# damemi/odigos

Measured on AMD Instinct MI355X. Metric: spans/sec processed (whole node) at 1/2/4/8 MI355X; % of HBM roofline, higher is better.
Workload: dtype u8; 1 GPU; C4: fused odigossampling -> odigosurltemplate -> odigostrafficmetrics, 100M spans in total (all on one GPU at N=1; ~100M/N per GPU, trace-id all-to-all over RCCL at N>1); spans_per_gpu=100000000, spans_total=100000000, template_form=refs, seed=219545604, parallelism=dp1: independent span shards, no data-path collective

## Files before the change

### odigos_amd/csrc/engine.cpp

```cpp
#include <hip/hip_runtime.h>

#include <algorithm>
#include <map>
#include <cstdio>
#include <cstdlib>
#include <cstring>
#include <mutex>
#include <string>
#include <unordered_map>
#include <vector>

#include "../../include/odigos_amd.h"
#include "config.hpp"
#include "devcfg.hpp"
#include "engine_internal.hpp"
#include "kernels.hpp"
#include "blob.hpp"
#include "regex_dfa.hpp"

namespace ose {

thread_local std::string g_last_error;

int fail(int code, const std::string& msg) {
// ... 134 lines not shown
    if (w->table) (void)hipFree(w->table);
    if (w->dup_bkt) (void)hipFree(w->dup_bkt);
    if (w->dup_bkt_count) (void)hipFree(w->dup_bkt_count);
    if (w->runs) (void)hipFree(w->runs);
    if (w->run_count) (void)hipFree(w->run_count);
    if (w->attr_bits) (void)hipFree(w->attr_bits);
    if (w->ep_planes) (void)hipFree(w->ep_planes);
    if (w->svc_local) (void)hipFree(w->svc_local);
    for (void* f : w->fold)
      if (f) (void)hipFree(f);
    if (w->pending) (void)hipEventDestroy(w->pending);
    if (w->dup_host) (void)hipHostFree(w->dup_host);
    if (w->dup_ready) (void)hipEventDestroy(w->dup_ready);
    if (w->fork) (void)hipEventDestroy(w->fork);
    if (w->join) (void)hipEventDestroy(w->join);
    delete w;
  }
}

hipEvent_t Engine::take_event() {
  if (!event_pool.empty()) {
    hipEvent_t ev = event_pool.back();
    event_pool.pop_back();
    return ev;
  }
  hipEvent_t ev = nullptr;
  (void)hipEventCreate(&ev);
  return ev;
}
void Engine::prof_begin(const char* name, hipStream_t st, Timed& t) {
// ... 46 lines not shown
  if (w->pending_set) (void)hipStreamWaitEvent(st, w->pending, 0);
  return w;
}
void Engine::return_unused_ws(Workspace* w) {
  std::lock_guard<std::mutex> g(mu);
  w->captured = false;
  free_ws.push_back(w);
}
void Engine::release_ws(Workspace* w, hipStream_t st) {
  if (w->captured) return;
  if (!w->pending) (void)hipEventCreateWithFlags(&w->pending, hipEventDisableTiming);
  w->pending_set = w->pending && hipEventRecord(w->pending, st) == hipSuccess;
  std::lock_guard<std::mutex> g(mu);
  free_ws.push_back(w);
}
hipStream_t Engine::take_stream() {
  std::lock_guard<std::mutex> g(mu);
  if (!free_streams.empty()) {
    hipStream_t s = free_streams.back();
    free_streams.pop_back();
    return s;
  }
  hipStream_t s = nullptr;
  if (hipStreamCreateWithFlags(&s, hipStreamNonBlocking) != hipSuccess) return nullptr;
  streams.push_back(s);
  return s;
}
void Engine::give_stream(hipStream_t s) {
  std::lock_guard<std::mutex> g(mu);
  free_streams.push_back(s);
}

int Workspace::reserve(size_t bytes) {
  if (bytes <= cap) return 0;
  if (captured) return fail(OSE_ENOMEM, "workspace too small inside a hipGraph capture: call ose_reserve first");
  if (dev) HIP_TRY(hipFree(dev));
  dev = nullptr;
  cap = 0;
  size_t want = std::max<size_t>(bytes, 1 << 20);
// ... 39 lines not shown
  (void)hipDeviceSynchronize();
  delete e;
}

int upload(const std::vector<uint8_t>& host, uint8_t** dev) {
  HIP_TRY(hipMalloc(dev, host.size()));
  HIP_TRY(hipMemcpy(*dev, host.data(), host.size(), hipMemcpyHostToDevice));
  return 0;
}

static size_t align_up(size_t x, size_t a) { return (x + a - 1) / a * a; }

int run_url_back(Engine* e, const UrlKernelArgs& a, hipStream_t st);

int run_url(Engine* e, const ose_columns* c, const ose_outputs* o, hipStream_t st, Workspace* ws, size_t ws_off = 0,
            UrlKernelArgs* front = nullptr, bool refs = false, uint32_t grid_mult = 1) {
  if (!e->has_url) return fail(OSE_EINVAL, "odigosurltemplate is not configured on this engine");
  if (!c->url_flags || !c->kind || !c->path || !c->arena || !o->url_out || !o->tmpl || !o->tmpl_arena)
    return fail(OSE_EINVAL, "TEMPLATE stage needs url_flags, kind, path, arena, url_out, tmpl, tmpl_arena");
  if (e->url_needs_resource && (!c->resource || !c->res_url_ok))
    return fail(OSE_EINVAL, "include/exclude configured: resource and res_url_ok columns are required");
  if (c->res_url_ok && !c->resource) return fail(OSE_EINVAL, "res_url_ok needs the resource column");
  if (o->tmpl_arena_cap > 0xFFFFFFFFull) return fail(OSE_ERANGE, "tmpl_arena_cap exceeds the 32-bit offset range");
  uint64_t n = c->n_spans;
  const uint32_t groups = (uint32_t)((n + kUrlGroup - 1) / kUrlGroup);
  const uint32_t scan_tiles = (groups + kUrlScanTile - 1) / kUrlScanTile;
  const size_t off_bump = 16, off_asum = 24, off_sst = 32, zero_bytes = off_sst + 8 * (size_t)scan_tiles;
  const size_t off_len = align_up(zero_bytes, 256), off_meta = off_len + 4 * n;
  const size_t off_code = align_up(off_meta + 4 * n, 8);
  const size_t off_gsum = off_code + 8 * n, off_gbase = off_gsum + 8 * (size_t)groups;
  const size_t off_gscr = off_gbase + 8 * (size_t)groups;
// ... 44 lines not shown
  a.slow_groups = reinterpret_cast<uint32_t*>(base + off_slow);
  a.unplanned_count = reinterpret_cast<uint32_t*>(base + 12);
  a.unplanned = reinterpret_cast<uint32_t*>(base + off_unpl);
  HIP_TRY(hipMemsetAsync(base, 0, zero_bytes, st));
  a.used = o->tmpl_arena_used;
#if OSE_DIAG
  if (const char* ab = getenv("OSE_URL_ABLATE")) a.ablate = (uint32_t)strtoul(ab, nullptr, 0);
#endif
  a.plan_grid_mult = refs ? grid_mult : 1u;
  a.scr_region = (scr_bytes / std::max<uint32_t>(1, url_plan_waves(a))) & ~15ull;
  a.plan_waves = url_plan_waves(a);
  a.refs_chunk = url_refs_chunk(o->tmpl_arena_cap, a.plan_waves);
  if (front) *front = a;
  if (n == 0) {
    if (o->tmpl_arena_used) HIP_TRY(hipMemsetAsync(o->tmpl_arena_used, 0, 8, st));
    return 0;
  }
  if (a.ablate & 512) {
    a.dbg = reinterpret_cast<uint64_t*>(base + off_dbg);
    HIP_TRY(hipMemsetAsync(a.dbg, 0, 256, st));
  }
  Engine::Timed tm{};
  e->prof_begin("url_plan_kernel", st, tm);
  launch_url_plan(a, st);
  HIP_TRY(hipGetLastError());
  e->prof_end(tm, st);
  e->prof_begin("url_plan_slow_kernel", st, tm);
  launch_url_plan_slow(a, st);
  HIP_TRY(hipGetLastError());
  e->prof_end(tm, st);
  e->prof_begin("url_scan_kernel", st, tm);
  launch_url_scan(a, st);
  HIP_TRY(hipGetLastError());
  e->prof_end(tm, st);
  e->prof_begin("url_emit_slow_kernel", st, tm);
  launch_url_emit_slow(a, st);
  HIP_TRY(hipGetLastError());
  e->prof_end(tm, st);
  if (front) {
    *front = a;
    return 0;
  }
  return run_url_back(e, a, st);
}

int run_url_back(Engine* e, const UrlKernelArgs& a, hipStream_t st) {
  if (a.n_spans == 0) return 0;
  Engine::Timed tm{};
  e->prof_begin("url_copy_kernel", st, tm);
  launch_url_copy(a, st);
  HIP_TRY(hipGetLastError());
  e->prof_end(tm, st);
  if (a.ablate & 512) {
    uint64_t h[16];
    uint32_t cnt[4];
    HIP_TRY(hipMemcpyAsync(h, a.dbg, sizeof h, hipMemcpyDeviceToHost, st));
    HIP_TRY(hipMemcpyAsync(cnt, a.scan_counter, sizeof cnt, hipMemcpyDeviceToHost, st));
    HIP_TRY(hipStreamSynchronize(st));
    const double wp = h[3] ? (double)h[3] : 1.0, we = h[6] ? (double)h[6] : 1.0;
    (void)we;
    fprintf(stderr, "url clocks/wave: plan[stage %.0f bitmaps %.0f plan %.0f assemble+store %.0f]\n", h[0] / wp,
            h[1] / wp, h[2] / wp, h[5] / wp);
    fprintf(stderr, "url plan list clocks/wave: enumerate %.0f classify %.0f fold %.0f\n", h[13] / wp, h[14] / wp,
            h[15] / wp);
    fprintf(stderr, "url groups: %llu, slow (K3s) %u, unplanned (K1b) %u\n", (unsigned long long)((a.n_spans + 63) / 64),
            cnt[1], cnt[3]);
    fprintf(stderr, "url_plan_slow_kernel slowest block clocks: config %llu whole %llu plan_path %llu\n",
// ... 30 lines not shown
  if (mask & OSE_STAGE_TEMPLATE) {
    need = std::max(need, url_off + url_workspace_bytes(n, c->arena_bytes));
    size_off = align_up(url_off + url_workspace_bytes(n, c->arena_bytes), 256);
  }
  if (mask & OSE_STAGE_SIZE) need = std::max(need, size_off + size_scratch_bytes(c->n_scopes, c->n_resources));
  int rc = ws->reserve(need);
  std::function<int()> sample_tail;
  UrlKernelArgs ua{};
  hipStream_t ust = nullptr;
  static const bool one_stream = getenv("OSE_ONE_STREAM") != nullptr;
  constexpr uint64_t kForkSpans = 1u << 20;
  const uint32_t plan_groups = (uint32_t)((n + kUrlGroup - 1) / kUrlGroup);
  if (!one_stream && !rc && defer && n >= kForkSpans) {
    if (!ws->fork) (void)hipEventCreateWithFlags(&ws->fork, hipEventDisableTiming);
    if (!ws->join) (void)hipEventCreateWithFlags(&ws->join, hipEventDisableTiming);
    if (ws->fork && ws->join) ust = e->take_stream();
    if (ust && (hipEventRecord(ws->fork, st) != hipSuccess || hipStreamWaitEvent(ust, ws->fork, 0) != hipSuccess)) {
      e->give_stream(ust);
      ust = nullptr;
    }
  }
  const bool tmpl = !rc && (mask & OSE_STAGE_TEMPLATE);
  ws->beside_url = ust && tmpl;
  if (ust && tmpl)
    rc = run_url(e, c, o, ust, ws, url_off, &ua, (mask & OSE_STAGE_TEMPLATE_REFS) != 0, url_plan_grid_mult(plan_groups, true));
  if (!rc && (mask & OSE_STAGE_SAMPLE)) rc = run_sampling(e, c, o, group_mode, rnd, st, ws, gate_on_host ? &sample_tail : nullptr);
  if (sample_tail && !defer) {
    rc = sample_tail();
    sample_tail = nullptr;
  }
  if (!ust && tmpl && !rc)
    rc = run_url(e, c, o, st, ws, url_off, &ua, (mask & OSE_STAGE_TEMPLATE_REFS) != 0, url_plan_grid_mult(plan_groups));
  if (sample_tail) {
    const int trc = sample_tail();
    if (!rc) rc = trc;
  }
  if (ust) {
    const hipError_t je = hipEventRecord(ws->join, ust);
    const hipError_t jw = je == hipSuccess ? hipStreamWaitEvent(st, ws->join, 0) : je;
    if (jw != hipSuccess) {
      (void)hipStreamSynchronize(ust);
      if (!rc) rc = fail(OSE_EDEVICE, std::string("URL stream join: ") + hipGetErrorString(jw));
    }
    e->give_stream(ust);
  }
  SizeKernelArgs sa{};
  bool size_on = false;
  if (!rc && (mask & OSE_STAGE_SIZE)) rc = prepare_size(e, c, o, mask, group_mode, rnd, st, ws, size_off, sa, size_on);
  if (!rc && tmpl) {
    if (size_on && n > 0 && !(OSE_DIAG && getenv("OSE_NO_FUSED_SIZE"))) {
      sa.kept_partials = size_partials_of(ws, size_off, c->n_scopes, c->n_resources);
      sa.n_kept_partials = url_copy_blocks(ua.n_groups);
      ua.fuse_size = 1;
      ua.size_partials = const_cast<uint32_t*>(sa.kept_partials);
      ua.sz = sa;
    }
    rc = run_url_back(e, ua, st);
  }
  if (!rc && size_on) rc = run_size_tail(e, sa, st);
  ws->beside_url = false;
  e->release_ws(ws, st);
  return rc;
}

}

using namespace ose;

extern "C" {

const char* ose_last_error(void) { return g_last_error.c_str(); }

uint64_t ose_dropped_errors(char* last, size_t cap) {
  std::lock_guard<std::mutex> g(g_dropped_mu);
// ... 312 lines not shown
```

### odigos_amd/csrc/engine_internal.hpp

```cpp
#pragma once
#include <hip/hip_runtime.h>

#include <atomic>
#include <cstdint>
#include <functional>
#include <mutex>
#include <string>
#include <unordered_map>
#include <vector>

#include "../../include/odigos_amd.h"
#include "config.hpp"

namespace ose {

int fail(int code, const std::string& msg);
struct Engine;
int bind_device(const Engine* e);
int ensure_device();
void engine_retain(Engine* e);
void engine_unref(Engine* e);
void note_dropped_error(const char* where, hipError_t err);
struct LastErrorScope {
  const char* where;
// ... 35 lines not shown
  uint64_t fold_cap = 0;
  int reserve_fold(uint64_t n_spans);
  uint64_t* attr_bits = nullptr;
  uint64_t attr_bits_cap = 0;
  int reserve_attr(uint64_t n_spans);
  uint64_t* ep_planes = nullptr;
  uint64_t ep_planes_cap = 0;
  ose_columns spill_cols{};
  uint32_t* svc_local = nullptr;
  uint64_t svc_local_cap = 0;
  ose_columns local_cols{};
  int reserve_svc_local(uint64_t n_resources);
  int reserve_ep_planes(uint64_t words);
  uint32_t* dup_host = nullptr;
  hipEvent_t dup_ready = nullptr;
  hipEvent_t fork = nullptr, join = nullptr;
  bool beside_url = false;
};

struct Engine {
  std::atomic<int> refs{1};
  std::atomic<bool> closed{false};
  int device = 0;
  UrlTemplateConfig url;
  SamplingConfig sampling;
  TrafficMetricsConfig traffic;
  bool has_url = false, has_sampling = false, has_traffic = false;
  enum : uint32_t { kOptOtlpGpuChain = 1, kOptOtlpHostResources = 2, kOptOtlpHostScopes = 4, kOptEncodeHost = 8 };
  std::atomic<uint32_t> options{0};
  bool option(uint32_t o) const { return (options.load(std::memory_order_relaxed) & o) != 0; }
  bool url_needs_resource = false;
// ... 83 lines not shown
```

### odigos_amd/csrc/size_kernel.hip

```cpp
#include <hip/hip_runtime.h>

#include <algorithm>
#include <cstdint>
#include <cstdlib>

#include "device_common.hpp"
#include "kernels.hpp"
#include "size_device.hpp"

namespace ose {
namespace {

using namespace sizedev;
constexpr int kSThreads = 256;
constexpr uint32_t kLdsAttrsets = 2048;

__device__ __forceinline__ bool batch_dropped(const SizeKernelArgs& a) { return size_batch_dropped(a); }

__global__ __launch_bounds__(kSThreads) void size_span_kernel(SizeKernelArgs a) {
  if (batch_dropped(a)) return;
  __shared__ uint32_t wk[kSThreads / kWave];
  uint32_t kept_total = 0;
  const uint64_t stride = (uint64_t)gridDim.x * kSThreads;
  for (uint64_t base = (uint64_t)blockIdx.x * kSThreads; base < a.n_spans; base += 2 * stride) {
    const SpanCols x0 = size_span_load(a, base + threadIdx.x);
    const SpanCols x1 = size_span_load(a, base + stride + threadIdx.x);
    kept_total += size_span_finish(a, x0);
    if (base + stride < a.n_spans) kept_total += size_span_finish(a, x1);
  }
#pragma unroll
// ... 6 lines not shown
    if (k) atomicAdd((unsigned long long*)a.accepted, (unsigned long long)k);
  }
}

__device__ __forceinline__ void size_finish_res(const SizeKernelArgs& a, unsigned long long* hist, bool lds, uint32_t r,
                                                uint64_t body, uint32_t alive, bool had, uint32_t rsz, uint32_t set) {
  const bool removed = a.remove_empty && had && alive == 0;
  const uint64_t size = removed ? 0 : (uint64_t)rsz + body;
  if (a.res_bytes) a.res_bytes[r] = size;
  if (removed) return;
  const long long add = (long long)size * a.inverse;
  if (lds) atomicAdd(&hist[set], (unsigned long long)add);
  else atomicAdd((unsigned long long*)&a.attrset_bytes[set], (unsigned long long)add);
}

__global__ __launch_bounds__(kSThreads) void size_tail_kernel(SizeKernelArgs a) {
  __shared__ unsigned long long hist[kLdsAttrsets];
  __shared__ uint32_t wk[kSThreads / kWave];
  const bool lds = a.n_attrsets <= kLdsAttrsets;
  const int lane = threadIdx.x & 63;
  const uint64_t gstride = (uint64_t)gridDim.x * kSThreads;
  if (batch_dropped(a)) {
    if (a.res_bytes)
      for (uint64_t r = (uint64_t)blockIdx.x * kSThreads + threadIdx.x; r < a.n_resources; r += gstride) a.res_bytes[r] = 0;
    return;
  }
  if (lds)
    for (uint32_t k = threadIdx.x; k < a.n_attrsets; k += kSThreads) hist[k] = 0;
  __syncthreads();
  const uint32_t S = a.n_scopes, R = a.n_resources;
  if (S == 0) {
    for (uint64_t r = (uint64_t)blockIdx.x * kSThreads + threadIdx.x; r < R; r += gstride)
      size_finish_res(a, hist, lds, (uint32_t)r, 0, 0, false, a.res_size[r], a.res_attrset[r]);
  }
  for (uint64_t t0 = (uint64_t)blockIdx.x * kSThreads; t0 < S; t0 += gstride) {
    const uint64_t s = t0 + threadIdx.x;
    const uint64_t s0 = s - lane;
    const bool valid = s < S;
    uint32_t r = 0xFFFFFFFFu, alive = 0, had = 0;
    uint64_t contrib = 0;
    uint32_t nb = 0xFFFFFFFFu;
    if (valid) {
      r = a.scope_resource[s];
      const uint64_t sb = a.scope_body[s];
      const uint64_t body = sb & kSumMask;
      had = (sb >> kSumBits) != 0;
      alive = !a.remove_empty || !had || body != 0;
      if (alive) contrib = field_len((uint64_t)a.scope_size[s] + body);
      if (lane == 0 && s > 0) nb = a.scope_resource[s - 1];
    }
    uint32_t rsz = 0, rset = 0;
    if (valid) {
      rsz = a.res_size[r];
      rset = a.res_attrset[r];
    }
    const uint64_t vmask = __ballot(valid);
    if (!vmask) continue;
    const int lastv = 63 - __clzll((long long)vmask);
    uint32_t na = 0xFFFFFFFFu;
    if (lane == lastv && s + 1 < S) na = a.scope_resource[s + 1];
    uint64_t v = contrib;
    uint32_t c = alive;
    const bool tail = wave_seg_sum(r, valid, v, c);
    const uint32_t pr = dpp_mov<0x138>(r, r);
    const bool head = valid && (lane == 0 || pr != r);
    const uint64_t heads = __ballot(head);
    const uint64_t hadm = __ballot(had != 0);
    const uint64_t upto = ~0ull >> (63 - lane);
    const int start = 63 - __clzll((long long)(heads & upto));
    const uint32_t h = (hadm & upto & (~0ull << start)) ? 1u : 0u;
    const uint32_t r0 = __builtin_amdgcn_readfirstlane(r);
    const uint32_t rl = (uint32_t)__builtin_amdgcn_readlane((int)r, lastv);
    const uint32_t before = __builtin_amdgcn_readfirstlane(nb);
    const uint32_t after = (uint32_t)__builtin_amdgcn_readlane((int)na, lastv);
    const bool whole_head = s0 == 0 || before != r0;
    const bool whole_tail = s0 + lastv + 1 >= S || after != rl;
    const int end0 = __builtin_ctzll(__ballot(tail));
    const bool single = end0 == lastv;
    const bool cut = tail && ((start == 0 && !whole_head) || (lane == lastv && !whole_tail));
    if (tail && !cut) size_finish_res(a, hist, lds, r, v, c, h != 0, rsz, rset);
    if (valid && head) {
      const uint32_t prev = lane ? pr : (s0 == 0 ? 0xFFFFFFFFu : before);
      for (uint32_t g = prev + 1; g < r; g++) size_finish_res(a, hist, lds, g, 0, 0, false, a.res_size[g], a.res_attrset[g]);
    }
    if (valid && s + 1 == S)
      for (uint32_t g = r + 1; g < R; g++) size_finish_res(a, hist, lds, g, 0, 0, false, a.res_size[g], a.res_attrset[g]);
    const uint64_t w = s0 >> 6;
    const uint32_t ch0 = (uint32_t)__builtin_amdgcn_readlane((int)(c | (h << 30)), end0);
    const uint64_t v0 = ((uint64_t)(uint32_t)__builtin_amdgcn_readlane((int)(uint32_t)(v >> 32), end0) << 32) |
                        (uint32_t)__builtin_amdgcn_readlane((int)(uint32_t)v, end0);
    const uint32_t chl = (uint32_t)__builtin_amdgcn_readlane((int)(c | (h << 30)), lastv);
    const uint64_t vl = ((uint64_t)(uint32_t)__builtin_amdgcn_readlane((int)(uint32_t)(v >> 32), lastv) << 32) |
                        (uint32_t)__builtin_amdgcn_readlane((int)(uint32_t)v, lastv);
    if (lane == 0 && valid) {
      a.parts[2 * w] = SizePart{r0, ch0 | (whole_head ? 1u << 31 : 0u), v0};
      a.parts[2 * w + 1] = SizePart{rl, chl | (whole_tail ? 1u << 31 : 0u), vl};
      a.fix[w] = (!whole_head && (!single || whole_tail)) ? 1u : 0u;
    }
  }
  if (a.kept_partials) {
    uint32_t k = 0;
    for (uint32_t b = blockIdx.x * kSThreads + threadIdx.x; b < a.n_kept_partials; b += gridDim.x * kSThreads)
      k += a.kept_partials[b];
#pragma unroll
    for (int o = 32; o > 0; o >>= 1) k += __shfl_xor(k, o, kWave);
    if (lane == 0) wk[threadIdx.x >> 6] = k;
    __syncthreads();
    if (threadIdx.x == 0) {
      uint32_t t = 0;
      for (int q = 0; q < kSThreads / kWave; q++) t += wk[q];
      if (t) atomicAdd((unsigned long long*)a.accepted, (unsigned long long)t);
    }
  }
// ... 17 lines not shown
    alive += lp.ch & 0x3FFFFFFFu;
    had |= (lp.ch >> 30) & 1u;
    const SizePart fp = a.parts[2 * k];
    if (fp.r != r || (fp.ch >> 31)) break;
  }
  size_finish_res(a, nullptr, false, r, body, alive, had, a.res_size[r], a.res_attrset[r]);
}
}

void launch_size_spans(const SizeKernelArgs& a, hipStream_t st) {
  constexpr uint64_t cap = 1024;
  const uint64_t blocks = std::min<uint64_t>((a.n_spans + kSThreads - 1) / kSThreads, cap);
  if (blocks) hipLaunchKernelGGL(size_span_kernel, dim3((uint32_t)blocks), dim3(kSThreads), 0, st, a);
}
void launch_size_tail(const SizeKernelArgs& a, hipStream_t st) {
  uint64_t blocks = ((uint64_t)a.n_scopes + kSThreads - 1) / kSThreads;
#ifndef OSE_SIZE_TAIL_CAP
#define OSE_SIZE_TAIL_CAP 4096
#endif
  if (blocks > OSE_SIZE_TAIL_CAP) blocks = OSE_SIZE_TAIL_CAP;
  if (a.kept_partials) blocks = std::max<uint64_t>(blocks, std::min<uint32_t>(64, (a.n_kept_partials + 4095) / 4096));
  if (!blocks && a.n_resources) blocks = std::min<uint64_t>(((uint64_t)a.n_resources + kSThreads - 1) / kSThreads, 1024);
  if (blocks) hipLaunchKernelGGL(size_tail_kernel, dim3((uint32_t)blocks), dim3(kSThreads), 0, st, a);
}
void launch_size_fix(const SizeKernelArgs& a, hipStream_t st) {
  if (a.n_swin) hipLaunchKernelGGL(size_fix_kernel, dim3((a.n_swin + kSThreads - 1) / kSThreads), dim3(kSThreads), 0, st, a);
}

}
```

### odigos_amd/csrc/url_kernel.hip

```cpp
#include <hip/hip_runtime.h>

#include <algorithm>
#include <cstdlib>

#include "../../include/odigos_amd.h"
#include "device_common.hpp"
#include "kernels.hpp"
#include "size_device.hpp"
#include "url_classes.hpp"

#ifndef OSE_ASM_BATCH
#define OSE_ASM_BATCH 0
#endif

namespace ose {
namespace {

constexpr int kThreads = 256;
constexpr int kWaves = kThreads / kWave;
constexpr uint32_t kStage = 4 * 1024;

enum : uint32_t { M_NONE = 0, M_RENAME_SLASH, M_SLASH, M_RULE, M_DEFAULT, M_ORIG };

__device__ __forceinline__ bool is_digit(uint32_t c) { return c - '0' < 10u; }
// ... 1358 lines not shown
      if (!(a.ablate & 64))
        assemble_group((lds_out_u8*)sm.bm[wv], L, (uint32_t)(stage - (uint8_t*)&sm), sm.segs[wv], sm.cls[wv], sm.bn,
                       bn_src, p, seg_off, local, cfg.n_custom == 0);
      wave_lds_sync();
      uint4* dst = reinterpret_cast<uint4*>(a.scratch + region + scr_used);
      for (uint32_t k = lane; k < n16; k += kWave) {
        const u32x4 v = img4[k];
        dst[k] = make_uint4(v.x, v.y, v.z, v.w);
      }
      if (lane == 0) {
        a.group_sum[g] = sum;
        a.group_scr[g] = region + scr_used;
      }
      if (a.refs && i < a.n_spans) a.tmpl[i] = ose_strref{(uint32_t)(region + scr_used + local), p.len};
      scr_used += need;
    } else if (lane == 0) {
      a.group_sum[g] = sum;
      a.group_scr[g] = ~0ull;
      if (sum) a.slow_groups[atomicAdd(a.slow_count, 1u)] = g;
    }
    }
    if (tm) { const uint64_t t1 = clk(); t_emit += t1 - t0; t0 = t1; }
    if (!more) break;
    wave_lds_sync();
    pf = stage_dma(a.arena, np2 ? nxt.pr.off : ~0u, np2 ? nxt.pr.off + nxt.pr.len : 0u, sm.stage[wv]);
    g = g2;
  }
  if (tm && lane == 0) {
    atomicAdd((unsigned long long*)&a.dbg[0], (unsigned long long)t_stage);
    atomicAdd((unsigned long long*)&a.dbg[1], (unsigned long long)t_bm);
    atomicAdd((unsigned long long*)&a.dbg[2], (unsigned long long)t_plan);
    atomicAdd((unsigned long long*)&a.dbg[3], 1ull);
    atomicAdd((unsigned long long*)&a.dbg[5], (unsigned long long)t_emit);
    atomicAdd((unsigned long long*)&a.dbg[13], (unsigned long long)tt[0]);
// ... 55 lines not shown
  }
  __syncthreads();
  if (k < a.n_groups) a.group_base[k] = sb + prefix + wbase + incl - v;
}

struct CopyCols {
  uint32_t len;
  uint64_t base, gsum, so;
};
__device__ __forceinline__ CopyCols copy_cols(const UrlKernelArgs& a, uint32_t g, int lane) {
  CopyCols c{0, 0, 0, ~0ull};
  const uint64_t i = (uint64_t)g * kWave + lane;
  c.base = a.group_base[g];
  c.gsum = a.group_sum[g];
  c.so = a.group_scr[g];
  if (i < a.n_spans) c.len = a.plan_len[i];
  return c;
}
__device__ __forceinline__ void copy_round(uint8_t* gdst, uint32_t shift, uint64_t endb, uint32_t c0, uint32_t nchunk,
                                           const uint4& v, uint32_t& carry) {
  const int lane = threadIdx.x & 63;
  const uint32_t c = c0 + (uint32_t)lane;
  uint32_t pw = (uint32_t)__shfl_up((int)v.w, 1, kWave);
  if (lane == 0) pw = carry;
  carry = lane_value(v.w, kWave - 1);
  const uint32_t sh = 4 - shift;
  const uint32_t w0 = shift ? __builtin_amdgcn_alignbyte(v.x, pw, sh) : v.x;
  const uint32_t w1 = shift ? __builtin_amdgcn_alignbyte(v.y, v.x, sh) : v.y;
  const uint32_t w2 = shift ? __builtin_amdgcn_alignbyte(v.z, v.y, sh) : v.z;
  const uint32_t w3 = shift ? __builtin_amdgcn_alignbyte(v.w, v.z, sh) : v.w;
// ... 10 lines not shown
#pragma unroll
      for (uint32_t q = 0; q < 16; q++)
        if (b0 + q >= shift && b0 + q < endb) gdst[b0 + q] = (uint8_t)(ws[q >> 2] >> (8 * (q & 3)));
    }
  }
}
struct CopyJob {
  const uint4* src;
  uint8_t* gdst;
  uint32_t shift, n16, nchunk;
  uint64_t endb;
  bool on;
};
__device__ __forceinline__ CopyJob copy_job(const UrlKernelArgs& a, const CopyCols& c) {
  CopyJob j{};
  j.on = !a.refs && c.so != ~0ull && c.gsum != 0 && c.base + c.gsum <= a.out_cap;
  if (!j.on) return j;
  j.src = reinterpret_cast<const uint4*>(a.scratch + c.so);
  j.shift = (uint32_t)(c.base & 3);
  j.gdst = a.out_arena + (c.base - j.shift);
  j.endb = j.shift + c.gsum;
  j.n16 = (uint32_t)((c.gsum + 15) / 16);
  j.nchunk = (uint32_t)((j.endb + 15) / 16);
  return j;
}
__device__ __forceinline__ uint4 copy_load(const CopyJob& j, uint32_t c0) {
  const uint32_t c = c0 + (threadIdx.x & 63);
  return j.on && c < j.n16 ? j.src[c] : make_uint4(0, 0, 0, 0);
}
__device__ __forceinline__ void copy_rest(const CopyJob& j, uint4 v, uint32_t& carry) {
  copy_round(j.gdst, j.shift, j.endb, 0, j.nchunk, v, carry);
  for (uint32_t c0 = kWave; c0 < j.nchunk; c0 += kWave) {
    v = copy_load(j, c0);
    copy_round(j.gdst, j.shift, j.endb, c0, j.nchunk, v, carry);
  }
}
template <bool kSize>
__global__ __launch_bounds__(kThreads) __attribute__((amdgpu_waves_per_eu(kSize ? 5 : 6, 8))) void url_copy_kernel(UrlKernelArgs a) {
  const int lane = threadIdx.x & 63;
  const uint32_t stride = wave_stride();
  if (!kSize && a.refs) {
    for (uint64_t g0 = (uint64_t)wave_first_group() * kWave; g0 < a.n_groups; g0 += (uint64_t)stride * kWave) {
      const uint64_t gg = g0 + lane;
      const bool other = gg < a.n_groups && a.group_scr[gg] == ~0ull;
      for (uint64_t m = __ballot(other); m; m &= m - 1) {
        const uint32_t g = (uint32_t)(g0 + __builtin_ctzll(m));
        const CopyCols A = copy_cols(a, g, lane);
        uint32_t unused;
        const uint32_t la = wave_excl_scan(A.len, &unused);
        const uint64_t ia = (uint64_t)g * kWave + lane;
        if (ia < a.n_spans) a.tmpl[ia] = ose_strref{(uint32_t)(A.base + la), A.len};
      }
    }
    return;
  }
  uint32_t kept = 0;
  const bool sz_on = kSize && !sizedev::size_batch_dropped(a.sz);
  uint32_t g = wave_first_group();
  CopyCols An{0, 0, 0, ~0ull};
  sizedev::SpanCols xn{};
  if (g < a.n_groups) {
    An = copy_cols(a, g, lane);
    if (kSize && sz_on) xn = sizedev::size_span_load(a.sz, (uint64_t)g * kWave + lane, false);
  }
  for (; g < a.n_groups; g += stride) {
    const uint64_t ia = (uint64_t)g * kWave + lane;
    const CopyCols A = An;
    const sizedev::SpanCols x0 = xn;
    const bool more = g + stride < a.n_groups;
    if (more) {
      An = copy_cols(a, g + stride, lane);
      if (kSize && sz_on) xn = sizedev::size_span_load(a.sz, (uint64_t)(g + stride) * kWave + lane, false);
    }
    sizedev::SpanCols x = x0;
    uint32_t unused;
    const uint32_t la = wave_excl_scan(A.len, &unused);
    const CopyJob ja = copy_job(a, A);
    const uint4 va = copy_load(ja, 0);
    if (ia < a.n_spans && !(a.refs && A.so != ~0ull)) {
      const uint64_t at = a.refs && A.so != ~0ull ? A.so : A.base;
      a.tmpl[ia] = ose_strref{(uint32_t)(at + la), A.len};
    }
    if (kSize && sz_on) {
      x.tl = A.len;
      kept += sizedev::size_span_finish(a.sz, x);
    }
    uint32_t carry = 0;
    if (ja.on) copy_rest(ja, va, carry);
    if (!more) break;
  }
  if (kSize) {
    __shared__ uint32_t wk[kWaves];
#pragma unroll
    for (int o = 32; o > 0; o >>= 1) kept += __shfl_xor(kept, o, kWave);
    if (lane == 0) wk[threadIdx.x >> 6] = kept;
    __syncthreads();
    if (threadIdx.x == 0) {
      uint32_t t = 0;
      for (int w = 0; w < kWaves; w++) t += wk[w];
      a.size_partials[blockIdx.x] = t;
    }
  }
}
// ... 70 lines not shown
      }
      wave_lds_sync();
      if (a.dbg) c_plan += clk() - t;
    }
    if (gate == 2) {
      oflags = OSE_OUT_SET_ATTR;
      if ((c.f & OSE_URL_NAME_EQ_METHOD) && p.len > 0) oflags |= OSE_OUT_RENAME;
    }
    if (i < a.n_spans) {
      a.plan_len[i] = p.len;
      a.url_out[i] = (uint8_t)oflags;
      a.plan_meta[i] = pack_meta(p.mode, p.lead, p.slow, oflags, p.field);
      a.plan_code[i] = p.code;
    }
    const uint64_t sum = wave_sum_u64(p.len);
    if (lane == 0) {
      a.group_sum[g] = sum;
      a.group_scr[g] = ~0ull;
      if (sum) a.slow_groups[atomicAdd(a.slow_count, 1u)] = g;
    }
  }
  if (a.dbg) {
    const uint64_t c2 = clk();
    if (lane == 0) {
      atomicMax((unsigned long long*)&a.dbg[8], (unsigned long long)(c1 - c0));
      atomicMax((unsigned long long*)&a.dbg[9], (unsigned long long)(c2 - c0));
      atomicMax((unsigned long long*)&a.dbg[10], (unsigned long long)c_plan);
    }
  }
}
// ... 5 lines not shown
};
__global__ __launch_bounds__(kThreads) void url_emit_slow_kernel(UrlKernelArgs a) {
  __shared__ EmitSlowSmem sm;
  const uint32_t count = *a.slow_count;
  if (blockIdx.x * kWaves >= count) return;
  const int lane = threadIdx.x & 63, wv = threadIdx.x >> 6;
  const Cfg cfg = load_cfg(a, sm.ns);
  uint8_t* stage = sm.stage[wv];
  lds_u32* stage32 = (lds_u32*)stage;
  lds_w32* img = (lds_w32*)sm.img[wv];
  for (uint32_t k = wave_first_group(); k < count; k += wave_stride()) {
    const uint32_t g = a.slow_groups[k];
    const uint64_t i = (uint64_t)g * kWave + lane;
    const EmitCols c = emit_cols(a, g, lane);
    const uint64_t base = c.base, gtotal = c.gsum;
    if (base + gtotal > a.out_cap) continue;
    const uint32_t len = c.len, meta = c.meta, mode = meta & 7u;
    uint32_t unused;
    const uint32_t local = wave_excl_scan(len, &unused);
    const bool needs_path = emit_needs_path(meta);
    const ose_strref pr = needs_path ? c.pr : ose_strref{0, 0};
    uint32_t nbytes;
    const uint32_t lo16 = stage_wave(stage, a.arena, needs_path ? pr.off : ~0u, needs_path ? pr.off + pr.len : 0u,
                                     &nbytes);
    const uint32_t shift = (uint32_t)(base & 3);
    const uint32_t img_bytes = shift + (uint32_t)gtotal;
    const bool direct = img_bytes > kWaveOut || lo16 == ~0u;
    if (!direct) {
      for (uint32_t k2 = lane; k2 < (img_bytes + 3) / 4; k2 += kWave) img[k2] = 0;
      wave_lds_sync();
    }
    if (len) {
      const uint32_t lead = (meta >> 3) & 1u, field = meta >> 7;
      const bool slow = (meta >> 4) & 1u;
// ... 61 lines not shown
#if OSE_DIAG
    case 2: launch_plan_mode<2>(a, st); break;
    case 3: launch_plan_mode<3>(a, st); break;
#endif
    default: launch_plan_mode<1>(a, st); break;
  }
}
void launch_url_scan(const UrlKernelArgs& a, hipStream_t st) {
  hipLaunchKernelGGL(url_scan_kernel, dim3(a.n_scan_tiles), dim3(kScanThreads), 0, st, a);
}
uint32_t url_copy_blocks(uint32_t n_groups) {
  return std::max<uint32_t>(1, std::min<uint32_t>(kUrlCopyMaxBlocks, (n_groups + 2 * kWaves - 1) / (2 * kWaves)));
}
void launch_url_copy(const UrlKernelArgs& a, hipStream_t st) {
  const uint32_t blocks = url_copy_blocks(a.n_groups);
  if (a.fuse_size)
    hipLaunchKernelGGL(url_copy_kernel<true>, dim3(blocks), dim3(kThreads), 0, st, a);
  else
    hipLaunchKernelGGL(url_copy_kernel<false>, dim3(blocks), dim3(kThreads), 0, st, a);
}
void launch_url_plan_slow(const UrlKernelArgs& a, hipStream_t st) {
  static const uint32_t cap = [] {
    int dev = 0, cus = 0, per_cu = 0;
    if (hipGetDevice(&dev) != hipSuccess) return 1024u;
    if (hipDeviceGetAttribute(&cus, hipDeviceAttributeMultiprocessorCount, dev) != hipSuccess || cus <= 0) cus = 256;
    if (hipOccupancyMaxActiveBlocksPerMultiprocessor(&per_cu, url_plan_slow_kernel, kWave, 0) != hipSuccess || per_cu <= 0)
      per_cu = 2;
    return (uint32_t)(cus * per_cu);
  }();
  const uint32_t blocks = std::min<uint32_t>(cap, a.n_groups);
  if (blocks) hipLaunchKernelGGL(url_plan_slow_kernel, dim3(blocks), dim3(kWave), 0, st, a);
}
void launch_url_emit_slow(const UrlKernelArgs& a, hipStream_t st) {
  static const uint32_t cap = resident_blocks(url_emit_slow_kernel, 0);
// ... 6 lines not shown
```

Measured before the change: 13.52 billion spans/s.

## Write template refs in plan/emit, drop refs copy pass, join URL stream early, batch size-tail loads

In the refs form, template references are now written directly by the plan, plan_slow and emit_slow kernels. The standalone refs pass in the copy kernel is removed, so in refs form the copy kernel runs only when fused size accounting needs span lengths. The main stream now waits on the side URL stream only after planning, via a new event, with a second join at the end, so more sampling work can overlap. The size tail kernel loads several tiles per block before processing them to raise memory-level parallelism, at the cost of more registers and a higher-priority side-stream option.

```diff
diff --git a/odigos_amd/csrc/engine.cpp b/odigos_amd/csrc/engine.cpp
--- a/odigos_amd/csrc/engine.cpp
+++ b/odigos_amd/csrc/engine.cpp
@@ -172,6 +172,7 @@
     if (w->dup_ready) (void)hipEventDestroy(w->dup_ready);
     if (w->fork) (void)hipEventDestroy(w->fork);
     if (w->join) (void)hipEventDestroy(w->join);
+    if (w->join2) (void)hipEventDestroy(w->join2);
     delete w;
   }
 }
@@ -248,6 +249,9 @@
   std::lock_guard<std::mutex> g(mu);
   free_ws.push_back(w);
 }
+#ifndef OSE_SIDE_STREAM_PRIO
+#define OSE_SIDE_STREAM_PRIO 0
+#endif
 hipStream_t Engine::take_stream() {
   std::lock_guard<std::mutex> g(mu);
   if (!free_streams.empty()) {
@@ -256,7 +260,13 @@
     return s;
   }
   hipStream_t s = nullptr;
+#if OSE_SIDE_STREAM_PRIO
+  int least = 0, greatest = 0;
+  (void)hipDeviceGetStreamPriorityRange(&least, &greatest);
+  if (hipStreamCreateWithPriority(&s, hipStreamNonBlocking, greatest) != hipSuccess) return nullptr;
+#else
   if (hipStreamCreateWithFlags(&s, hipStreamNonBlocking) != hipSuccess) return nullptr;
+#endif
   streams.push_back(s);
   return s;
 }
@@ -326,7 +336,7 @@
 int run_url_back(Engine* e, const UrlKernelArgs& a, hipStream_t st);
 
 int run_url(Engine* e, const ose_columns* c, const ose_outputs* o, hipStream_t st, Workspace* ws, size_t ws_off = 0,
-            UrlKernelArgs* front = nullptr, bool refs = false, uint32_t grid_mult = 1) {
+            UrlKernelArgs* front = nullptr, bool refs = false, uint32_t grid_mult = 1, hipEvent_t planned = nullptr) {
   if (!e->has_url) return fail(OSE_EINVAL, "odigosurltemplate is not configured on this engine");
   if (!c->url_flags || !c->kind || !c->path || !c->arena || !o->url_out || !o->tmpl || !o->tmpl_arena)
     return fail(OSE_EINVAL, "TEMPLATE stage needs url_flags, kind, path, arena, url_out, tmpl, tmpl_arena");
@@ -401,6 +411,7 @@
   if (front) *front = a;
   if (n == 0) {
     if (o->tmpl_arena_used) HIP_TRY(hipMemsetAsync(o->tmpl_arena_used, 0, 8, st));
+    if (planned) HIP_TRY(hipEventRecord(planned, st));
     return 0;
   }
   if (a.ablate & 512) {
@@ -416,6 +427,7 @@
   launch_url_plan_slow(a, st);
   HIP_TRY(hipGetLastError());
   e->prof_end(tm, st);
+  if (planned) HIP_TRY(hipEventRecord(planned, st));
   e->prof_begin("url_scan_kernel", st, tm);
   launch_url_scan(a, st);
   HIP_TRY(hipGetLastError());
@@ -433,11 +445,13 @@
 
 int run_url_back(Engine* e, const UrlKernelArgs& a, hipStream_t st) {
   if (a.n_spans == 0) return 0;
-  Engine::Timed tm{};
-  e->prof_begin("url_copy_kernel", st, tm);
-  launch_url_copy(a, st);
-  HIP_TRY(hipGetLastError());
-  e->prof_end(tm, st);
+  if (!a.refs || a.fuse_size) {
+    Engine::Timed tm{};
+    e->prof_begin("url_copy_kernel", st, tm);
+    launch_url_copy(a, st);
+    HIP_TRY(hipGetLastError());
+    e->prof_end(tm, st);
+  }
   if (a.ablate & 512) {
     uint64_t h[16];
     uint32_t cnt[4];
@@ -498,7 +512,8 @@
   if (!one_stream && !rc && defer && n >= kForkSpans) {
     if (!ws->fork) (void)hipEventCreateWithFlags(&ws->fork, hipEventDisableTiming);
     if (!ws->join) (void)hipEventCreateWithFlags(&ws->join, hipEventDisableTiming);
-    if (ws->fork && ws->join) ust = e->take_stream();
+    if (!ws->join2) (void)hipEventCreateWithFlags(&ws->join2, hipEventDisableTiming);
+    if (ws->fork && ws->join && ws->join2) ust = e->take_stream();
     if (ust && (hipEventRecord(ws->fork, st) != hipSuccess || hipStreamWaitEvent(ust, ws->fork, 0) != hipSuccess)) {
       e->give_stream(ust);
       ust = nullptr;
@@ -506,8 +521,17 @@
   }
   const bool tmpl = !rc && (mask & OSE_STAGE_TEMPLATE);
   ws->beside_url = ust && tmpl;
-  if (ust && tmpl)
-    rc = run_url(e, c, o, ust, ws, url_off, &ua, (mask & OSE_STAGE_TEMPLATE_REFS) != 0, url_plan_grid_mult(plan_groups, true));
+  bool early_join = false;
+#ifndef OSE_URL_JOIN_LATE
+  early_join = ust && tmpl && !rc && (mask & OSE_STAGE_TEMPLATE_REFS) && (mask & OSE_STAGE_SIZE) &&
+               !(OSE_DIAG && getenv("OSE_NO_FUSED_SIZE"));
+#endif
+  bool join_recorded = false;
+  if (ust && tmpl && !rc) {
+    rc = run_url(e, c, o, ust, ws, url_off, &ua, (mask & OSE_STAGE_TEMPLATE_REFS) != 0, url_plan_grid_mult(plan_groups, true),
+                 early_join ? ws->join : nullptr);
+    join_recorded = early_join && !rc;
+  }
   if (!rc && (mask & OSE_STAGE_SAMPLE)) rc = run_sampling(e, c, o, group_mode, rnd, st, ws, gate_on_host ? &sample_tail : nullptr);
   if (sample_tail && !defer) {
     rc = sample_tail();
@@ -520,13 +544,12 @@
     if (!rc) rc = trc;
   }
   if (ust) {
-    const hipError_t je = hipEventRecord(ws->join, ust);
+    const hipError_t je = join_recorded ? hipSuccess : hipEventRecord(ws->join, ust);
     const hipError_t jw = je == hipSuccess ? hipStreamWaitEvent(st, ws->join, 0) : je;
     if (jw != hipSuccess) {
       (void)hipStreamSynchronize(ust);
       if (!rc) rc = fail(OSE_EDEVICE, std::string("URL stream join: ") + hipGetErrorString(jw));
     }
-    e->give_stream(ust);
   }
   SizeKernelArgs sa{};
   bool size_on = false;
@@ -542,6 +565,17 @@
     rc = run_url_back(e, ua, st);
   }
   if (!rc && size_on) rc = run_size_tail(e, sa, st);
+  if (ust) {
+    if (join_recorded) {
+      const hipError_t je = hipEventRecord(ws->join2, ust);
+      const hipError_t jw = je == hipSuccess ? hipStreamWaitEvent(st, ws->join2, 0) : je;
+      if (jw != hipSuccess) {
+        (void)hipStreamSynchronize(ust);
+        if (!rc) rc = fail(OSE_EDEVICE, std::string("URL stream join: ") + hipGetErrorString(jw));
+      }
+    }
+    e->give_stream(ust);
+  }
   ws->beside_url = false;
   e->release_ws(ws, st);
   return rc;
diff --git a/odigos_amd/csrc/engine_internal.hpp b/odigos_amd/csrc/engine_internal.hpp
--- a/odigos_amd/csrc/engine_internal.hpp
+++ b/odigos_amd/csrc/engine_internal.hpp
@@ -73,7 +73,7 @@
   int reserve_ep_planes(uint64_t words);
   uint32_t* dup_host = nullptr;
   hipEvent_t dup_ready = nullptr;
-  hipEvent_t fork = nullptr, join = nullptr;
+  hipEvent_t fork = nullptr, join = nullptr, join2 = nullptr;
   bool beside_url = false;
 };
 
diff --git a/odigos_amd/csrc/size_kernel.hip b/odigos_amd/csrc/size_kernel.hip
--- a/odigos_amd/csrc/size_kernel.hip
+++ b/odigos_amd/csrc/size_kernel.hip
@@ -14,6 +14,10 @@
 using namespace sizedev;
 constexpr int kSThreads = 256;
 constexpr uint32_t kLdsAttrsets = 2048;
+#ifndef OSE_SIZE_TAIL_TILES
+#define OSE_SIZE_TAIL_TILES 4
+#endif
+constexpr int kTailTiles = OSE_SIZE_TAIL_TILES;
 
 __device__ __forceinline__ bool batch_dropped(const SizeKernelArgs& a) { return size_batch_dropped(a); }
 
@@ -50,6 +54,96 @@
   else atomicAdd((unsigned long long*)&a.attrset_bytes[set], (unsigned long long)add);
 }
 
+struct TailCols {
+  uint64_t s, sb, vmask;
+  uint32_t r, ssz, nb, na, rsz, rset;
+  bool valid;
+};
+__device__ __forceinline__ TailCols size_tail_load(const SizeKernelArgs& a, uint64_t s) {
+  const int lane = threadIdx.x & 63;
+  const uint32_t S = a.n_scopes;
+  TailCols x{};
+  x.s = s;
+  x.valid = s < S;
+  x.r = 0xFFFFFFFFu;
+  x.nb = 0xFFFFFFFFu;
+  x.na = 0xFFFFFFFFu;
+  x.vmask = __ballot(x.valid);
+  if (x.valid) {
+    x.r = a.scope_resource[s];
+    x.sb = a.scope_body[s];
+    x.ssz = a.scope_size[s];
+    if (lane == 0 && s > 0) x.nb = a.scope_resource[s - 1];
+    if (s + 1 < S && !((x.vmask >> 1) >> lane)) x.na = a.scope_resource[s + 1];
+  }
+  return x;
+}
+__device__ __forceinline__ void size_tail_gather(const SizeKernelArgs& a, TailCols& x) {
+  if (x.valid) {
+    x.rsz = a.res_size[x.r];
+    x.rset = a.res_attrset[x.r];
+  }
+}
+
+__device__ __forceinline__ void size_tail_window(const SizeKernelArgs& a, unsigned long long* hist, bool lds,
+                                                 const TailCols& x) {
+  const uint64_t vmask = x.vmask;
+  if (!vmask) return;
+  const int lane = threadIdx.x & 63;
+  const uint32_t S = a.n_scopes, R = a.n_resources;
+  const uint64_t s = x.s;
+  const uint64_t s0 = s - lane;
+  const bool valid = x.valid;
+  const uint32_t r = x.r;
+  uint32_t alive = 0, had = 0;
+  uint64_t contrib = 0;
+  if (valid) {
+    const uint64_t body = x.sb & kSumMask;
+    had = (x.sb >> kSumBits) != 0;
+    alive = !a.remove_empty || !had || body != 0;
+    if (alive) contrib = field_len((uint64_t)x.ssz + body);
+  }
+  const int lastv = 63 - __clzll((long long)vmask);
+  uint64_t v = contrib;
+  uint32_t c = alive;
+  const bool tail = wave_seg_sum(r, valid, v, c);
+  const uint32_t pr = dpp_mov<0x138>(r, r);
+  const bool head = valid && (lane == 0 || pr != r);
+  const uint64_t heads = __ballot(head);
+  const uint64_t hadm = __ballot(had != 0);
+  const uint64_t upto = ~0ull >> (63 - lane);
+  const int start = 63 - __clzll((long long)(heads & upto));
+  const uint32_t h = (hadm & upto & (~0ull << start)) ? 1u : 0u;
+  const uint32_t r0 = __builtin_amdgcn_readfirstlane(r);
+  const uint32_t rl = (uint32_t)__builtin_amdgcn_readlane((int)r, lastv);
+  const uint32_t before = __builtin_amdgcn_readfirstlane(x.nb);
+  const uint32_t after = (uint32_t)__builtin_amdgcn_readlane((int)x.na, lastv);
+  const bool whole_head = s0 == 0 || before != r0;
+  const bool whole_tail = s0 + lastv + 1 >= S || after != rl;
+  const int end0 = __builtin_ctzll(__ballot(tail));
+  const bool single = end0 == lastv;
+  const bool cut = tail && ((start == 0 && !whole_head) || (lane == lastv && !whole_tail));
+  if (tail && !cut) size_finish_res(a, hist, lds, r, v, c, h != 0, x.rsz, x.rset);
+  if (valid && head) {
+    const uint32_t prev = lane ? pr : (s0 == 0 ? 0xFFFFFFFFu : before);
+    for (uint32_t g = prev + 1; g < r; g++) size_finish_res(a, hist, lds, g, 0, 0, false, a.res_size[g], a.res_attrset[g]);
+  }
+  if (valid && s + 1 == S)
+    for (uint32_t g = r + 1; g < R; g++) size_finish_res(a, hist, lds, g, 0, 0, false, a.res_size[g], a.res_attrset[g]);
+  const uint64_t w = s0 >> 6;
+  const uint32_t ch0 = (uint32_t)__builtin_amdgcn_readlane((int)(c | (h << 30)), end0);
+  const uint64_t v0 = ((uint64_t)(uint32_t)__builtin_amdgcn_readlane((int)(uint32_t)(v >> 32), end0) << 32) |
+                      (uint32_t)__builtin_amdgcn_readlane((int)(uint32_t)v, end0);
+  const uint32_t chl = (uint32_t)__builtin_amdgcn_readlane((int)(c | (h << 30)), lastv);
+  const uint64_t vl = ((uint64_t)(uint32_t)__builtin_amdgcn_readlane((int)(uint32_t)(v >> 32), lastv) << 32) |
+                      (uint32_t)__builtin_amdgcn_readlane((int)(uint32_t)v, lastv);
+  if (lane == 0 && valid) {
+    a.parts[2 * w] = SizePart{r0, ch0 | (whole_head ? 1u << 31 : 0u), v0};
+    a.parts[2 * w + 1] = SizePart{rl, chl | (whole_tail ? 1u << 31 : 0u), vl};
+    a.fix[w] = (!whole_head && (!single || whole_tail)) ? 1u : 0u;
+  }
+}
+
 __global__ __launch_bounds__(kSThreads) void size_tail_kernel(SizeKernelArgs a) {
   __shared__ unsigned long long hist[kLdsAttrsets];
   __shared__ uint32_t wk[kSThreads / kWave];
@@ -69,70 +163,14 @@
     for (uint64_t r = (uint64_t)blockIdx.x * kSThreads + threadIdx.x; r < R; r += gstride)
       size_finish_res(a, hist, lds, (uint32_t)r, 0, 0, false, a.res_size[r], a.res_attrset[r]);
   }
-  for (uint64_t t0 = (uint64_t)blockIdx.x * kSThreads; t0 < S; t0 += gstride) {
-    const uint64_t s = t0 + threadIdx.x;
-    const uint64_t s0 = s - lane;
-    const bool valid = s < S;
-    uint32_t r = 0xFFFFFFFFu, alive = 0, had = 0;
-    uint64_t contrib = 0;
-    uint32_t nb = 0xFFFFFFFFu;
-    if (valid) {
-      r = a.scope_resource[s];
-      const uint64_t sb = a.scope_body[s];
-      const uint64_t body = sb & kSumMask;
-      had = (sb >> kSumBits) != 0;
-      alive = !a.remove_empty || !had || body != 0;
-      if (alive) contrib = field_len((uint64_t)a.scope_size[s] + body);
-      if (lane == 0 && s > 0) nb = a.scope_resource[s - 1];
-    }
-    uint32_t rsz = 0, rset = 0;
-    if (valid) {
-      rsz = a.res_size[r];
-      rset = a.res_attrset[r];
-    }
-    const uint64_t vmask = __ballot(valid);
-    if (!vmask) continue;
-    const int lastv = 63 - __clzll((long long)vmask);
-    uint32_t na = 0xFFFFFFFFu;
-    if (lane == lastv && s + 1 < S) na = a.scope_resource[s + 1];
-    uint64_t v = contrib;
-    uint32_t c = alive;
-    const bool tail = wave_seg_sum(r, valid, v, c);
-    const uint32_t pr = dpp_mov<0x138>(r, r);
-    const bool head = valid && (lane == 0 || pr != r);
-    const uint64_t heads = __ballot(head);
-    const uint64_t hadm = __ballot(had != 0);
-    const uint64_t upto = ~0ull >> (63 - lane);
-    const int start = 63 - __clzll((long long)(heads & upto));
-    const uint32_t h = (hadm & upto & (~0ull << start)) ? 1u : 0u;
-    const uint32_t r0 = __builtin_amdgcn_readfirstlane(r);
-    const uint32_t rl = (uint32_t)__builtin_amdgcn_readlane((int)r, lastv);
-    const uint32_t before = __builtin_amdgcn_readfirstlane(nb);
-    const uint32_t after = (uint32_t)__builtin_amdgcn_readlane((int)na, lastv);
-    const bool whole_head = s0 == 0 || before != r0;
-    const bool whole_tail = s0 + lastv + 1 >= S || after != rl;
-    const int end0 = __builtin_ctzll(__ballot(tail));
-    const bool single = end0 == lastv;
-    const bool cut = tail && ((start == 0 && !whole_head) || (lane == lastv && !whole_tail));
-    if (tail && !cut) size_finish_res(a, hist, lds, r, v, c, h != 0, rsz, rset);
-    if (valid && head) {
-      const uint32_t prev = lane ? pr : (s0 == 0 ? 0xFFFFFFFFu : before);
-      for (uint32_t g = prev + 1; g < r; g++) size_finish_res(a, hist, lds, g, 0, 0, false, a.res_size[g], a.res_attrset[g]);
-    }
-    if (valid && s + 1 == S)
-      for (uint32_t g = r + 1; g < R; g++) size_finish_res(a, hist, lds, g, 0, 0, false, a.res_size[g], a.res_attrset[g]);
-    const uint64_t w = s0 >> 6;
-    const uint32_t ch0 = (uint32_t)__builtin_amdgcn_readlane((int)(c | (h << 30)), end0);
-    const uint64_t v0 = ((uint64_t)(uint32_t)__builtin_amdgcn_readlane((int)(uint32_t)(v >> 32), end0) << 32) |
-                        (uint32_t)__builtin_amdgcn_readlane((int)(uint32_t)v, end0);
-    const uint32_t chl = (uint32_t)__builtin_amdgcn_readlane((int)(c | (h << 30)), lastv);
-    const uint64_t vl = ((uint64_t)(uint32_t)__builtin_amdgcn_readlane((int)(uint32_t)(v >> 32), lastv) << 32) |
-                        (uint32_t)__builtin_amdgcn_readlane((int)(uint32_t)v, lastv);
-    if (lane == 0 && valid) {
-      a.parts[2 * w] = SizePart{r0, ch0 | (whole_head ? 1u << 31 : 0u), v0};
-      a.parts[2 * w + 1] = SizePart{rl, chl | (whole_tail ? 1u << 31 : 0u), vl};
-      a.fix[w] = (!whole_head && (!single || whole_tail)) ? 1u : 0u;
-    }
+  for (uint64_t t0 = (uint64_t)blockIdx.x * kSThreads; t0 < S; t0 += kTailTiles * gstride) {
+    TailCols x[kTailTiles];
+#pragma unroll
+    for (int j = 0; j < kTailTiles; j++) x[j] = size_tail_load(a, t0 + j * gstride + threadIdx.x);
+#pragma unroll
+    for (int j = 0; j < kTailTiles; j++) size_tail_gather(a, x[j]);
+#pragma unroll
+    for (int j = 0; j < kTailTiles; j++) size_tail_window(a, hist, lds, x[j]);
   }
   if (a.kept_partials) {
     uint32_t k = 0;
@@ -180,7 +218,8 @@
   if (blocks) hipLaunchKernelGGL(size_span_kernel, dim3((uint32_t)blocks), dim3(kSThreads), 0, st, a);
 }
 void launch_size_tail(const SizeKernelArgs& a, hipStream_t st) {
-  uint64_t blocks = ((uint64_t)a.n_scopes + kSThreads - 1) / kSThreads;
+  const uint64_t tiles = ((uint64_t)a.n_scopes + kSThreads - 1) / kSThreads;
+  uint64_t blocks = (tiles + kTailTiles - 1) / kTailTiles;
 #ifndef OSE_SIZE_TAIL_CAP
 #define OSE_SIZE_TAIL_CAP 4096
 #endif
diff --git a/odigos_amd/csrc/url_kernel.hip b/odigos_amd/csrc/url_kernel.hip
--- a/odigos_amd/csrc/url_kernel.hip
+++ b/odigos_amd/csrc/url_kernel.hip
@@ -1396,10 +1396,13 @@
       }
       if (a.refs && i < a.n_spans) a.tmpl[i] = ose_strref{(uint32_t)(region + scr_used + local), p.len};
       scr_used += need;
-    } else if (lane == 0) {
-      a.group_sum[g] = sum;
-      a.group_scr[g] = ~0ull;
-      if (sum) a.slow_groups[atomicAdd(a.slow_count, 1u)] = g;
+    } else {
+      if (a.refs && sum == 0 && i < a.n_spans) a.tmpl[i] = ose_strref{0, 0};
+      if (lane == 0) {
+        a.group_sum[g] = sum;
+        a.group_scr[g] = ~0ull;
+        if (sum) a.slow_groups[atomicAdd(a.slow_count, 1u)] = g;
+      }
     }
     }
     if (tm) { const uint64_t t1 = clk(); t_emit += t1 - t0; t0 = t1; }
@@ -1485,6 +1488,12 @@
   c.base = a.group_base[g];
   c.gsum = a.group_sum[g];
   c.so = a.group_scr[g];
+  if (i < a.n_spans) c.len = a.plan_len[i];
+  return c;
+}
+__device__ __forceinline__ CopyCols copy_len(const UrlKernelArgs& a, uint32_t g, int lane) {
+  CopyCols c{0, 0, 0, ~0ull};
+  const uint64_t i = (uint64_t)g * kWave + lane;
   if (i < a.n_spans) c.len = a.plan_len[i];
   return c;
 }
@@ -1525,7 +1534,7 @@
 };
 __device__ __forceinline__ CopyJob copy_job(const UrlKernelArgs& a, const CopyCols& c) {
   CopyJob j{};
-  j.on = !a.refs && c.so != ~0ull && c.gsum != 0 && c.base + c.gsum <= a.out_cap;
+  j.on = c.so != ~0ull && c.gsum != 0 && c.base + c.gsum <= a.out_cap;
   if (!j.on) return j;
   j.src = reinterpret_cast<const uint4*>(a.scratch + c.so);
   j.shift = (uint32_t)(c.base & 3);
@@ -1546,32 +1555,19 @@
     copy_round(j.gdst, j.shift, j.endb, c0, j.nchunk, v, carry);
   }
 }
-template <bool kSize>
+template <bool kSize, bool kRefs>
 __global__ __launch_bounds__(kThreads) __attribute__((amdgpu_waves_per_eu(kSize ? 5 : 6, 8))) void url_copy_kernel(UrlKernelArgs a) {
+  static_assert(kSize || !kRefs, "the refs form has no copy pass");
   const int lane = threadIdx.x & 63;
   const uint32_t stride = wave_stride();
-  if (!kSize && a.refs) {
-    for (uint64_t g0 = (uint64_t)wave_first_group() * kWave; g0 < a.n_groups; g0 += (uint64_t)stride * kWave) {
-      const uint64_t gg = g0 + lane;
-      const bool other = gg < a.n_groups && a.group_scr[gg] == ~0ull;
-      for (uint64_t m = __ballot(other); m; m &= m - 1) {
-        const uint32_t g = (uint32_t)(g0 + __builtin_ctzll(m));
-        const CopyCols A = copy_cols(a, g, lane);
-        uint32_t unused;
-        const uint32_t la = wave_excl_scan(A.len, &unused);
-        const uint64_t ia = (uint64_t)g * kWave + lane;
-        if (ia < a.n_spans) a.tmpl[ia] = ose_strref{(uint32_t)(A.base + la), A.len};
-      }
-    }
-    return;
-  }
   uint32_t kept = 0;
   const bool sz_on = kSize && !sizedev::size_batch_dropped(a.sz);
   uint32_t g = wave_first_group();
+  if (kRefs && !sz_on) g = a.n_groups;
   CopyCols An{0, 0, 0, ~0ull};
   sizedev::SpanCols xn{};
   if (g < a.n_groups) {
-    An = copy_cols(a, g, lane);
+    An = kRefs ? copy_len(a, g, lane) : copy_cols(a, g, lane);
     if (kSize && sz_on) xn = sizedev::size_span_load(a.sz, (uint64_t)g * kWave + lane, false);
   }
   for (; g < a.n_groups; g += stride) {
@@ -1580,24 +1576,25 @@
     const sizedev::SpanCols x0 = xn;
     const bool more = g + stride < a.n_groups;
     if (more) {
-      An = copy_cols(a, g + stride, lane);
+      An = kRefs ? copy_len(a, g + stride, lane) : copy_cols(a, g + stride, lane);
       if (kSize && sz_on) xn = sizedev::size_span_load(a.sz, (uint64_t)(g + stride) * kWave + lane, false);
     }
     sizedev::SpanCols x = x0;
-    uint32_t unused;
-    const uint32_t la = wave_excl_scan(A.len, &unused);
-    const CopyJob ja = copy_job(a, A);
-    const uint4 va = copy_load(ja, 0);
-    if (ia < a.n_spans && !(a.refs && A.so != ~0ull)) {
-      const uint64_t at = a.refs && A.so != ~0ull ? A.so : A.base;
-      a.tmpl[ia] = ose_strref{(uint32_t)(at + la), A.len};
+    CopyJob ja{};
+    uint4 va = make_uint4(0, 0, 0, 0);
+    if (!kRefs) {
+      uint32_t unused;
+      const uint32_t la = wave_excl_scan(A.len, &unused);
+      ja = copy_job(a, A);
+      va = copy_load(ja, 0);
+      if (ia < a.n_spans) a.tmpl[ia] = ose_strref{(uint32_t)(A.base + la), A.len};
     }
     if (kSize && sz_on) {
       x.tl = A.len;
       kept += sizedev::size_span_finish(a.sz, x);
     }
     uint32_t carry = 0;
-    if (ja.on) copy_rest(ja, va, carry);
+    if (!kRefs && ja.on) copy_rest(ja, va, carry);
     if (!more) break;
   }
   if (kSize) {
@@ -1698,6 +1695,7 @@
       a.plan_code[i] = p.code;
     }
     const uint64_t sum = wave_sum_u64(p.len);
+    if (a.refs && sum == 0 && i < a.n_spans) a.tmpl[i] = ose_strref{0, 0};
     if (lane == 0) {
       a.group_sum[g] = sum;
       a.group_scr[g] = ~0ull;
@@ -1733,10 +1731,11 @@
     const uint64_t i = (uint64_t)g * kWave + lane;
     const EmitCols c = emit_cols(a, g, lane);
     const uint64_t base = c.base, gtotal = c.gsum;
-    if (base + gtotal > a.out_cap) continue;
     const uint32_t len = c.len, meta = c.meta, mode = meta & 7u;
     uint32_t unused;
     const uint32_t local = wave_excl_scan(len, &unused);
+    if (a.refs && i < a.n_spans) a.tmpl[i] = ose_strref{(uint32_t)(base + local), len};
+    if (base + gtotal > a.out_cap) continue;
     const bool needs_path = emit_needs_path(meta);
     const ose_strref pr = needs_path ? c.pr : ose_strref{0, 0};
     uint32_t nbytes;
@@ -1828,10 +1827,13 @@
 }
 void launch_url_copy(const UrlKernelArgs& a, hipStream_t st) {
   const uint32_t blocks = url_copy_blocks(a.n_groups);
-  if (a.fuse_size)
-    hipLaunchKernelGGL(url_copy_kernel<true>, dim3(blocks), dim3(kThreads), 0, st, a);
-  else
-    hipLaunchKernelGGL(url_copy_kernel<false>, dim3(blocks), dim3(kThreads), 0, st, a);
+  if (a.refs) {
+    if (a.fuse_size) hipLaunchKernelGGL((url_copy_kernel<true, true>), dim3(blocks), dim3(kThreads), 0, st, a);
+  } else if (a.fuse_size) {
+    hipLaunchKernelGGL((url_copy_kernel<true, false>), dim3(blocks), dim3(kThreads), 0, st, a);
+  } else {
+    hipLaunchKernelGGL((url_copy_kernel<false, false>), dim3(blocks), dim3(kThreads), 0, st, a);
+  }
 }
 void launch_url_plan_slow(const UrlKernelArgs& a, hipStream_t st) {
   static const uint32_t cap = [] {
```

New measurement: 14.10 billion spans/s (median of 6 runs). +4.3%, better.
